# akashsengupta1997/indirect_learning_pose-shape

Hardware: AMD Instinct MI355X
Metric: meshes/sec fwd+bwd (SMPL->48x48 31-part seg) (higher is better)
Workload: dtype f32; 1 GPU; full decoder fwd+bwd (batch_smpl + projection + compute_mask + projects_to_seg), BASELINE configs[2]; meshes_per_gpu=128, global_batch=128, img_wh=48, vertex_sampling=1, verts=6890, params_per_mesh=86, launch=graph, steps_per_graph_launch=10, concurrent_chunks=1

## Files before the change

indirect_learning_pose-shape_amd/csrc/seg_bin.hip:

```cpp
#include "raster_common.h"

namespace smplr {
constexpr int BIN_Q0 = 3;
constexpr float X_ZERO = 104.0f;
constexpr float M_LOCAL = 208.0f;
#ifdef SMPLR_TL
constexpr int TL_BIN_WG = 128;
__device__ unsigned g_tl_bin[TL_BIN_WG * (BIN_T / 64) * 32];
#endif

struct Slot {
  int cls;
  int pos, pix;
  float u, v, m, x;
};

__device__ __forceinline__ Slot classify(float u, float v, float m, int pos, int W) {
  Slot s;
  s.pos = pos;
  s.u = u;
  s.v = v;
  s.m = m;
  s.cls = 1;
  s.pix = 0;
  s.x = 0.f;
  if (s.m > M_LOCAL) {
    s.cls = 0;
    const float c = rintf(s.u), r = rintf(s.v);
    if (c >= 0.0f && c <= (float)(W - 1) && r >= 0.0f && r <= (float)(W - 1)) {
      const float du = s.u - c, dv = s.v - r;
      s.x = __builtin_amdgcn_sqrtf(fmaf(du, du, dv * dv) * (s.m * s.m));
      if (s.x < X_ZERO) {
        s.cls = 2;
        s.pix = (int)r * W + (int)c;
      }
    }
  }
  return s;
}

template <bool VIS, bool STAGE, bool SKIN>
__global__ __launch_bounds__(BIN_T) void seg_bin_kernel(const float *__restrict__ proj,
                                                        float *__restrict__ mask,
                                                        const int *__restrict__ part_pos,
                                                        const int *__restrict__ part_off, int P, int K,
                                                        int VP, int W, int S, float4 *__restrict__ G,
                                                        int *__restrict__ goff, int *__restrict__ lstart,
                                                        uint2 *__restrict__ lrec, int vgrid, int ref_compat,
                                                        short *__restrict__ vslot, SkinIn sk) {
  extern __shared__ __attribute__((aligned(16))) int s_cnt[];
  __shared__ int s_poff[33], s_gstart[33], s_gpad[33], s_wave[BIN_T / 64], s_gb[BIN_T];
  __shared__ int s_any_empty, s_nonunit;
  __shared__ float4 sAj[SKIN ? 72 : 1];
  static_assert(!SKIN || (VIS && STAGE), "the skinning form is built for the decoder's path only");
  const int n = blockIdx.x, tid = threadIdx.x;
  SMPLR_TL_WAVE(g_tl_bin, BIN_T / 64, n, TL_BIN_WG)
  const int npix = W * W;
  const float *pj = proj + (size_t)n * VP * 3;
  float *mk = mask + (size_t)n * VP;
  const int cells = VIS ? vgrid * vgrid : 0, words = VIS ? (VP + 31) / 32 : 0;
  unsigned long long *zbuf = reinterpret_cast<unsigned long long *>(s_cnt + ((npix + 1) & ~1));
  unsigned int *vis = reinterpret_cast<unsigned int *>(zbuf + cells);
  float *sU = reinterpret_cast<float *>(vis + words), *sV = sU + VP;
  short *vsl = vslot ? vslot + (size_t)n * VP : nullptr;

  const int ipt = (K + BIN_T - 1) / BIN_T;
  const int k0 = tid * ipt, k1 = min(K, k0 + ipt);
  int pos[IPT_MAX];
  if (!SKIN) {
#pragma unroll
    for (int j = 0; j < IPT_MAX; ++j) pos[j] = (j < ipt) ? part_pos[min(k0 + j, K - 1)] : 0;
  }
  constexpr int VPT = SKIN ? 7 : 8;
  float vu[VPT], vv[VPT], vz[VPT];
  float4 tw[SKIN ? VPT : 1], tj[SKIN ? VPT : 1], aj = {0.f, 0.f, 0.f, 0.f};
  float c0 = 0.f, c1 = 0.f, c2 = 0.f, c3 = 0.f;
  if (SKIN) {
    aj = reinterpret_cast<const float4 *>(sk.A + (size_t)n * 288)[tid < 72 ? tid : 71];
    const float *c = sk.cam + (size_t)n * sk.x_stride;
    c0 = c[0]; c1 = c[1]; c2 = c[2]; c3 = c[3];
    const float *vp = sk.v_posed + (size_t)n * VP * 3;
#pragma unroll
    for (int q = 0; q < BIN_Q0; ++q) {
      const int v = min(tid + q * BIN_T, VP - 1);
      const float4 *tp = reinterpret_cast<const float4 *>(sk.top4 + (size_t)v * 8);
      tw[q] = tp[0];
      tj[q] = tp[1];
      vu[q] = vp[v * 3 + 0];
      vv[q] = vp[v * 3 + 1];
      vz[q] = vp[v * 3 + 2];
    }
  } else if (VIS || STAGE) {
#pragma unroll
    for (int q = 0; q < VPT; ++q) {
      const int v = min(tid + q * BIN_T, VP - 1);
      vu[q] = pj[v * 3 + 0];
      vv[q] = pj[v * 3 + 1];
      vz[q] = VIS ? pj[v * 3 + 2] : 0.0f;
    }
  }
  if (tid <= P) s_poff[tid] = part_off[tid];
  if (tid == 0) { s_nonunit = 0; s_any_empty = 0; }
  for (int i = tid; i < npix; i += BIN_T) s_cnt[i] = 0;
  if (vslot && !SKIN)
    for (int i = tid; i < VP; i += BIN_T) vsl[i] = -1;
  if (VIS) {
    for (int i = tid; i < cells; i += BIN_T) zbuf[i] = 0ull;
    for (int i = tid; i < words; i += BIN_T) vis[i] = 0u;
  }
  if (SKIN && tid < 72) sAj[tid] = aj;
  SMPLR_TL_STAMP(1);
  __syncthreads();
  SMPLR_TL_STAMP(2);
  if (SKIN) {
    const float *vp = sk.v_posed + (size_t)n * VP * 3;
#pragma unroll
    for (int q = BIN_Q0; q < VPT; ++q) {
      const int v = min(tid + q * BIN_T, VP - 1);
      const float4 *tp = reinterpret_cast<const float4 *>(sk.top4 + (size_t)v * 8);
      tw[q] = tp[0];
      tj[q] = tp[1];
      vu[q] = vp[v * 3 + 0];
      vv[q] = vp[v * 3 + 1];
      vz[q] = vp[v * 3 + 2];
    }
    if (vslot)
      for (int i = tid; i < VP; i += BIN_T) vsl[i] = -1;
    __builtin_amdgcn_sched_barrier(0);
    float *vo = sk.verts + (size_t)n * VP * 3, *po = sk.proj + (size_t)n * VP * 3;
#pragma unroll
    for (int q = 0; q < VPT; ++q) {
      const int v = tid + q * BIN_T;
      float T[12], X, Y, Z;
      skin_T_sparse(sAj, tw[q], tj[q], T);
      skin_apply(T, vu[q], vv[q], vz[q], X, Y, Z);
      vu[q] = project_u(X, c0, c2);
      vv[q] = project_u(Y, c1, c3);
      vz[q] = Z;
      if (v < VP) {
        if (sk.verts) { SMPLR_OUT_STORE(&vo[v * 3 + 0], X); SMPLR_OUT_STORE(&vo[v * 3 + 1], Y); SMPLR_OUT_STORE(&vo[v * 3 + 2], Z); }
        if (sk.proj) { SMPLR_OUT_STORE(&po[v * 3 + 0], vu[q]); SMPLR_OUT_STORE(&po[v * 3 + 1], vv[q]); SMPLR_OUT_STORE(&po[v * 3 + 2], Z); }
      }
      __builtin_amdgcn_sched_barrier(0);
    }
#pragma unroll
    for (int j = 0; j < IPT_MAX; ++j) pos[j] = (j < ipt) ? part_pos[min(k0 + j, K - 1)] : 0;
  }
  if (VIS || STAGE) {
    const float fG = (float)vgrid;
    for (int base = 0; base < VP; base += VPT * BIN_T) {
      if (base > 0) {
#pragma unroll
        for (int q = 0; q < VPT; ++q) {
          const int v = min(base + tid + q * BIN_T, VP - 1);
          vu[q] = pj[v * 3 + 0];
          vv[q] = pj[v * 3 + 1];
          vz[q] = VIS ? pj[v * 3 + 2] : 0.0f;
        }
      }
#pragma unroll
      for (int q = 0; q < VPT; ++q) {
        const int v = base + tid + q * BIN_T;
        if (v < VP) {
          if (STAGE) { sU[v] = vu[q]; sV[v] = vv[q]; }
          if (VIS) {
            const float pu = rintf(vu[q]);
            const float pv = rintf(vv[q]);
            if (pu >= 0.0f && pu < fG && pv >= 0.0f && pv < fG) {
              const int cell = (int)pv * vgrid + (int)pu;
              const unsigned long long key = ((unsigned long long)orderable(vz[q]) << 32) |
                                             (unsigned long long)(0xFFFFFFFFu - (unsigned)v);
              atomicMax(&zbuf[cell], key);
            }
          }
        }
      }
    }
    SMPLR_TL_STAMP(3);
    __syncthreads();
    SMPLR_TL_STAMP(4);
  }
  bool vertex1 = false;
  if (VIS) {
    int empty = 0;
    for (int i = tid; i < cells; i += BIN_T) {
      const unsigned long long key = zbuf[i];
      if (key == 0ull) {
        empty = 1;
      } else {
        const unsigned int v = 0xFFFFFFFFu - (unsigned int)(key & 0xFFFFFFFFull);
        atomicOr(&vis[v >> 5], 1u << (v & 31));
      }
    }
    if (empty) s_any_empty = 1;
    SMPLR_TL_STAMP(5);
    __syncthreads();
    SMPLR_TL_STAMP(6);
    vertex1 = s_any_empty && ref_compat && VP > 1;
    if (mask)
      for (int v = tid; v < VP; v += BIN_T)
        SMPLR_OUT_STORE(&mk[v], (((vis[v >> 5] >> (v & 31)) & 1u) || (vertex1 && v == 1)) ? 1.0f : 500.0f);
  }
  SMPLR_TL_STAMP(7);
  float4 *Gn = G + (size_t)n * S;
  int *goffn = goff + (size_t)n * goff_stride(P);
  int *lstartn = lstart + (size_t)n * (npix + 1);
  uint2 *lrecn = lrec + (size_t)n * K;

  Slot sl[IPT_MAX];
  int gcnt = 0;
  unsigned gbits = 0;
#pragma unroll
  for (int j = 0; j < IPT_MAX; ++j) {
    const int k = k0 + j;
    sl[j].cls = 0;
    if (j < ipt && k < k1) {
      const int ps = pos[j];
      const float m = VIS ? ((((vis[ps >> 5] >> (ps & 31)) & 1u) || (vertex1 && ps == 1)) ? 1.0f : 500.0f) : mk[ps];
      const float u = STAGE ? sU[ps] : pj[ps * 3], v = STAGE ? sV[ps] : pj[ps * 3 + 1];
      sl[j] = classify(u, v, m, ps, W);
    }
    if (sl[j].cls == 1) {
      ++gcnt;
      gbits |= 1u << j;
      if (sl[j].m != 1.0f) s_nonunit = 1;
    } else if (sl[j].cls == 2) {
      atomicAdd(&s_cnt[sl[j].pix], 1);
    }
  }
  int p0 = 0;
  if (k0 < k1) {
    int lo = 0, hi = P;
    while (hi - lo > 1) {
      const int mid = (lo + hi) >> 1;
      if (s_poff[mid] <= k0) lo = mid; else hi = mid;
    }
    p0 = lo;
  }
  SMPLR_TL_STAMP(8);
  __syncthreads();
  SMPLR_TL_STAMP(9);
  const int ept = (npix + BIN_T - 1) / BIN_T;
  const int e0 = tid * ept, e1 = min(npix, e0 + ept);
  int loc = 0;
  for (int e = e0; e < e1; ++e) loc += s_cnt[e];
  int tot2;
  const int base2 = block_excl_scan(gcnt | (loc << 16), s_wave, &tot2);
  const int gbase = base2 & 0xffff, gtotal = tot2 & 0xffff, ltotal = tot2 >> 16;
  SMPLR_TL_STAMP(10);
  s_gb[tid] = gbase | (int)(gbits << 16);
  {
    int run = base2 >> 16;
    for (int e = e0; e < e1; ++e) {
      const int c = s_cnt[e];
      s_cnt[e] = run;
      lstartn[e] = run;
      run += c;
    }
    if (tid == 0) lstartn[npix] = ltotal;
  }
  SMPLR_TL_STAMP(11);
  __syncthreads();
  SMPLR_TL_STAMP(12);
  if (tid < 128) {
    const int l = tid & 63;
    int gs = gtotal;
    const int kk = s_poff[l <= P ? l : P];
    if (l < P && kk < K) {
      const int t = kk / ipt, j = kk - t * ipt;
      const int w = s_gb[t];
      gs = (w & 0xffff) + __popc(((unsigned)w >> 16) & ((1u << j) - 1u));
    }
    const int gnext = __shfl_down(gs, 1, 64);
    const int cnt = (l < P) ? (gnext - gs + GP - 1) / GP * GP : 0;
    if (tid < 64) {
      int inc = cnt;
#pragma unroll
      for (int o = 1; o < 32; o <<= 1) {
        const int t = __shfl_up(inc, o, 64);
        if (tid >= o) inc += t;
      }
      if (tid <= P) {
        s_gstart[tid] = gs;
        s_gpad[tid] = inc - cnt;
        goffn[tid] = inc - cnt;
      }
    } else {
      const int key = l < P ? ((cnt << 5) | (31 - l)) : -1;
      int rank = 0;
#pragma unroll
      for (int q = 0; q < 31; ++q) rank += (__builtin_amdgcn_readlane(key, q) > key) ? 1 : 0;
      if (l < P) goffn[P + 2 + rank] = l;
    }
  }
  SMPLR_TL_STAMP(13);
  __syncthreads();
  SMPLR_TL_STAMP(14);
  {
    int p = p0;
    int run = gbase;
#pragma unroll
    for (int j = 0; j < IPT_MAX; ++j) {
      const int k = k0 + j;
      if (!(j < ipt && k < k1)) continue;
      while (k >= s_poff[p + 1]) ++p;
      const Slot s = sl[j];
      if (s.cls == 1) {
        const int slot = s_gpad[p] + (run - s_gstart[p]);
        Gn[slot] = make_float4(s.u, s.v, s.m * s.m, __int_as_float(s.pos));
        if (vslot) vsl[s.pos] = (short)slot;
        ++run;
      } else if (s.cls == 2) {
        const int dst = atomicAdd(&s_cnt[s.pix], 1);
        lrecn[dst] = make_uint2(__float_as_uint(s.x), (unsigned)p);
        Gn[s_gpad[P] + dst] = make_float4(s.u, s.v, s.m * s.m, __int_as_float(s.pos));
        if (vslot) vsl[s.pos] = (short)(s_gpad[P] + dst);
      }
    }
  }
  SMPLR_TL_STAMP(15);
  if (tid == 0) goffn[P + 1] = s_nonunit;
  if (tid == 0)
    Gn[S - 1] = make_float4(__int_as_float(s_gpad[P] + lstartn[npix]), __int_as_float(s_nonunit), __int_as_float(s_gpad[P]),
                            __int_as_float(-1));
  if (tid < P) {
    const int cnt = s_gstart[tid + 1] - s_gstart[tid];
    for (int i = s_gpad[tid] + cnt; i < s_gpad[tid + 1]; ++i)
      Gn[i] = make_float4(INFINITY, INFINITY, 1.0f, __int_as_float(-1));
  }
  SMPLR_TL_STAMP(16);
  SMPLR_TL_STAMP(17);
  SMPLR_TL_STAMP(18);
}

struct BinLds { size_t base, total; bool stage; };
static BinLds bin_lds(int VP, int W, int grid_wh ) {
  BinLds b;
  b.base = (size_t)((W * W + 1) & ~1) * sizeof(int);
  if (grid_wh > 0) b.base += (size_t)grid_wh * grid_wh * 8 + (size_t)((VP + 31) / 32) * 4;
  b.stage = b.base + (size_t)VP * 8 <= 150 * 1024;
  b.total = b.base + (b.stage ? (size_t)VP * 8 : 0);
  return b;
}

int seg_bin_impl(const char *fn, const float *proj, float *mask, bool fuse_vis, int grid_wh, int ref_compat, int B, int VP,
                 int W, const int32_t *part_pos, const int32_t *part_off, int P, int K, void *workspace, float *rec,
                 int16_t *vslot, void *stream, SkinIn sk) {
  SMPLR_REQUIRE(B >= 0 && VP > 0 && VP <= 32767 && W > 0 && W <= 160 && P >= 1 && P <= 31 && K > 0 && K <= BIN_T * IPT_MAX,
                "%s: bad sizes B=%d VP=%d W=%d (max 160) P=%d (max 31) K=%d", fn, B, VP, W, P, K);
  SMPLR_REQUIRE(!fuse_vis || (grid_wh > 0 && grid_wh <= 128), "%s: bad grid_wh=%d (max 128)", fn, grid_wh);
  if (B == 0) return 0;
  const bool skin = sk.v_posed != nullptr;
  SMPLR_REQUIRE((skin || (proj && mask)) && part_pos && part_off && workspace && rec, "%s: null pointer", fn);
  SMPLR_REQUIRE(!skin || (sk.top4 && sk.A && sk.cam && sk.x_stride >= 4 && sk.proj == proj && fuse_vis &&
                          VP <= 7 * BIN_T),
                "%s: the skinning form needs the sparse weights, A, camera rows, the fused mask and V <= %d",
                fn, 7 * BIN_T);
  hipStream_t st = as_stream(stream);
  const SegWs ws = seg_ws_layout(B, W, P, K);
  const int S = seg_slots(P, K);
  char *base = reinterpret_cast<char *>(workspace);
  float4 *G = reinterpret_cast<float4 *>(rec);
  int *goff = reinterpret_cast<int *>(base + ws.goff_off);
  int *lstart = reinterpret_cast<int *>(base + ws.lstart_off);
  uint2 *lrec = reinterpret_cast<uint2 *>(base + ws.lrec_off);
  const BinLds bl = bin_lds(VP, W, fuse_vis ? grid_wh : 0);
  SMPLR_REQUIRE(bl.base <= 150 * 1024, "%s: pixel counters + grid + flags need %zu B of LDS (max 153600)", fn, bl.base);
  const bool stage = bl.stage;
  const size_t lds = bl.total;
#define SMPLR_BIN_LAUNCH(VIS_, STAGE_, SKIN_)                                                                 \
  {                                                                                                           \
    int rc = lds_attr<&seg_bin_kernel<VIS_, STAGE_, SKIN_>>(lds);          \
    if (rc) return rc;                                                                                        \
    hipLaunchKernelGGL((seg_bin_kernel<VIS_, STAGE_, SKIN_>), dim3(B), dim3(BIN_T), lds, st, proj, mask,      \
                       part_pos, part_off, P, K, VP, W, S, G, goff, lstart, lrec, fuse_vis ? grid_wh : 1,     \
                       ref_compat, reinterpret_cast<short *>(vslot), sk);                                     \
  }
  SMPLR_REQUIRE(!skin || stage, "%s: the skinning form needs the staged (u, v) to fit LDS", fn);
  if (skin) SMPLR_BIN_LAUNCH(true, true, true)
  else if (fuse_vis && stage) SMPLR_BIN_LAUNCH(true, true, false)
  else if (fuse_vis) SMPLR_BIN_LAUNCH(true, false, false)
  else if (stage) SMPLR_BIN_LAUNCH(false, true, false)
  else SMPLR_BIN_LAUNCH(false, false, false)
#undef SMPLR_BIN_LAUNCH
  SMPLR_LAUNCH_CHECK(fn);
  return 0;
}
}

extern "C" {

int smplr_seg_slots(int P, int K) { return (P > 0 && K > 0) ? smplr::seg_slots(P, K) : 0; }

size_t smplr_seg_workspace(int B, int VP, int W, int P, int K) {
  if (B <= 0 || VP <= 0 || W <= 0 || P <= 0 || K <= 0) return 0;
  return smplr::seg_ws_layout(B, W, P, K).total;
}

int smplr_seg_bin(const float *proj, float *mask, int B, int VP, int W, int grid_wh, int ref_compat,
                  const int32_t *part_pos, const int32_t *part_off, int P, int K, void *workspace, float *rec,
                  int16_t *vslot, void *stream) {
  return smplr::seg_bin_impl("smplr_seg_bin", proj, mask, grid_wh > 0, grid_wh, ref_compat, B, VP, W, part_pos,
                             part_off, P, K, workspace, rec, vslot, stream);
}

int smplr_skin_vis_seg_fits(int V, int W, int grid_wh) {
  if (V <= 0 || V > 7 * smplr::BIN_T || W <= 0 || W > 160 || grid_wh <= 0 || grid_wh > 128) return 0;
  const smplr::BinLds b = smplr::bin_lds(V, W, grid_wh);
  return (b.base <= 150 * 1024 && b.stage) ? 1 : 0;
}

}

#ifdef SMPLR_TL
SMPLR_TL_EXPORT(bin, smplr::g_tl_bin, smplr::TL_BIN_WG * (smplr::BIN_T / 64) * 32)
#endif
```

indirect_learning_pose-shape_amd/csrc/skin.hip:

```cpp
#include "common.h"

namespace smplr {

typedef float f32x4 __attribute__((ext_vector_type(4)));

constexpr int SK_MB = 1;
constexpr int SKB_T = 256;

template <bool SPARSE>
__global__ __launch_bounds__(256) void skin_fwd_kernel(const float *__restrict__ v_posed,
                                                       const float *__restrict__ lbs,
                                                       const float *__restrict__ top4,
                                                       const float *__restrict__ A,
                                                       const float *__restrict__ cam, int x_stride,
                                                       int B, int V, int vs, int VP,
                                                       float *__restrict__ verts,
                                                       float *__restrict__ proj) {
  __shared__ float4 sAj[SPARSE ? 72 : 1];
  const int v = blockIdx.x * 256 + threadIdx.x;
  const bool live = v < V;
  const int vc = live ? v : V - 1;
  float w[SPARSE ? 1 : 24];
  float4 ww = {0.f, 0.f, 0.f, 0.f}, jj = {0.f, 0.f, 0.f, 0.f};
  if (SPARSE) {
// ... 141 lines not shown
    if (slot >= 0) { gp0 += sx; gp1 += sy; }
  }
  if (tid < 72) sAj[tid] = aj;
  SMPLR_TL_STAMP(1);
  __syncthreads();
  SMPLR_TL_STAMP(2);

  const int cr = li >> 2, cc = li & 3;

  {
    const bool proj_on = live && has_proj && sampled;
    float g0 = 0.f, g1 = 0.f, g2 = 0.f;
    float dku = 0.f, dkv = 0.f, du0 = 0.f, dv0 = 0.f;
    if (live) { g0 = gv0; g1 = gv1; g2 = gv2; }
    if (proj_on) { g0 = fmaf(ck0, gp0, g0); g1 = fmaf(ck1, gp1, g1); g2 += gp2; du0 = gp0; dv0 = gp1; }
    float dp0 = 0.f, dp1 = 0.f, dp2 = 0.f;
#pragma unroll
    for (int r = 0; r < 3; ++r) {
      float t0 = 0.f, t1 = 0.f, t2 = 0.f, t3 = 0.f;
#pragma unroll
      for (int jq = 0; jq < (SPARSE ? 4 : 24); ++jq) {
        const int j = SPARSE ? jx[jq & 3] : jq;
        const float wj = SPARSE ? w4[jq & 3] : w[SPARSE ? 0 : jq];
        const float4 rr = sAj[j * 3 + r];
        t0 = fmaf(wj, rr.x, t0); t1 = fmaf(wj, rr.y, t1); t2 = fmaf(wj, rr.z, t2); t3 = fmaf(wj, rr.w, t3);
      }
      const float gr = r == 0 ? g0 : (r == 1 ? g1 : g2);
      dp0 = fmaf(t0, gr, dp0); dp1 = fmaf(t1, gr, dp1); dp2 = fmaf(t2, gr, dp2);
      if (r < 2 && proj_on) {
        const float XY = fmaf(t2, p2, fmaf(t1, p1, fmaf(t0, p0, t3)));
        if (r == 0) dku = XY * gp0; else dkv = XY * gp1;
      }
    }
    if (live) {
      float *o = dv_posed + ((size_t)n * V + v) * 3;
      o[0] = dp0; o[1] = dp1; o[2] = dp2;
    }
    SMPLR_TL_STAMP(3);
    float wa0[8], wa1[8];
    const __amdgpu_buffer_rsrc_t rs =
        __builtin_amdgcn_make_buffer_rsrc(const_cast<float *>(lbs), 0, V * 24 * 4, 0x00020000);
    const int vb = blockIdx.x * SKB_T + wave * 64 + lk;
    const int o0 = (vb * 24 + li) * 4, o1 = (vb * 24 + 16 + (li & 7)) * 4;
    {
  #pragma unroll
      for (int sI = 0; sI < 8; ++sI) {
        wa0[sI] = __builtin_bit_cast(float, __builtin_amdgcn_raw_buffer_load_b32(rs, o0 + sI * 384, 0, 0));
        wa1[sI] = __builtin_bit_cast(float, __builtin_amdgcn_raw_buffer_load_b32(rs, o1 + sI * 384, 0, 0));
      }
    }
    sG[tid][0] = g0; sG[tid][1] = g1; sG[tid][2] = g2; sG[tid][3] = 0.f;
    sP[tid][0] = p0; sP[tid][1] = p1; sP[tid][2] = p2; sP[tid][3] = 1.0f;
    __syncthreads();
    SMPLR_TL_STAMP(4);

    f32x4 acc0 = {0.f, 0.f, 0.f, 0.f}, acc1 = {0.f, 0.f, 0.f, 0.f};
#pragma unroll
    for (int s = 0; s < 16; ++s) {
      const int t = wave * 64 + s * 4 + lk;
      const float a0 = wa0[s & 7];
      const float a1 = (li < 8) ? wa1[s & 7] : 0.0f;
      const float b = (li < 12) ? sG[t][cr] * sP[t][cc] : 0.0f;
      acc0 = __builtin_amdgcn_mfma_f32_16x16x4f32(a0, b, acc0, 0, 0, 0);
      acc1 = __builtin_amdgcn_mfma_f32_16x16x4f32(a1, b, acc1, 0, 0, 0);
      if (s < 8) {
        wa0[s] = __builtin_bit_cast(float, __builtin_amdgcn_raw_buffer_load_b32(rs, o0 + (s + 8) * 384, 0, 0));
        wa1[s] = __builtin_bit_cast(float, __builtin_amdgcn_raw_buffer_load_b32(rs, o1 + (s + 8) * 384, 0, 0));
      }
    }
    SMPLR_TL_STAMP(5);
    if (li < 12) {
#pragma unroll
      for (int r = 0; r < 4; ++r) {
        const int j0 = lk * 4 + r;
        sRed[wave][j0 * 12 + li] = acc0[r];
        if (j0 < 8) sRed[wave][(16 + j0) * 12 + li] = acc1[r];
      }
    }
    const float r0 = wave_sum(dku), r1 = wave_sum(dkv), r2 = wave_sum(du0), r3 = wave_sum(dv0);
    if (lane == 0) {
      sRed[wave][288] = r0; sRed[wave][289] = r1; sRed[wave][290] = r2; sRed[wave][291] = r3;
    }
    __syncthreads();
    SMPLR_TL_STAMP(6);
    for (int e = tid; e < SKB_PART; e += SKB_T) {
      float acc = 0.f;
#pragma unroll
      for (int wv = 0; wv < SKB_T / 64; ++wv) acc += sRed[wv][e];
      part[((size_t)n * gridDim.x + blockIdx.x) * SKB_PART + e] = acc;
    }
    SMPLR_TL_STAMP(7);
  }
}

__global__ __launch_bounds__(320) void skin_bwd_reduce_kernel(const float *__restrict__ part, int nblk,
                                                              float *__restrict__ dA,
                                                              float *__restrict__ dcam) {
  const int n = blockIdx.x, e = threadIdx.x;
  if (e >= SKB_PART) return;
  float acc = 0.f;
  for (int b = 0; b < nblk; ++b) acc += part[((size_t)n * nblk + b) * SKB_PART + e];
  if (e < 288) dA[(size_t)n * 288 + e] = acc;
  else if (dcam) dcam[(size_t)n * 4 + (e - 288)] = acc;
}

__global__ __launch_bounds__(256) void project_fwd_kernel(const float *__restrict__ verts,
                                                          const float *__restrict__ cam, int x_stride,
                                                          int V, int vs, int VP, float *__restrict__ proj) {
  const int n = blockIdx.y, i = blockIdx.x * 256 + threadIdx.x;
  if (i >= VP) return;
  const float *c = cam + (size_t)n * x_stride;
  const float *p = verts + ((size_t)n * V + (size_t)i * vs) * 3;
  float *o = proj + ((size_t)n * VP + i) * 3;
  o[0] = c[2] + p[0] * c[0];
  o[1] = c[3] + p[1] * c[1];
  o[2] = p[2];
}

__global__ __launch_bounds__(256) void project_bwd_kernel(const float *__restrict__ dproj,
                                                          const float *__restrict__ verts,
                                                          const float *__restrict__ cam, int x_stride,
                                                          int V, int vs, int VP, float *__restrict__ dverts,
                                                          float *__restrict__ dcam) {
  __shared__ float red[4][4];
  const int n = blockIdx.x, tid = threadIdx.x;
  const float *c = cam + (size_t)n * x_stride;
  const float ku = c[0], kv = c[1];
  float s0 = 0.f, s1 = 0.f, s2 = 0.f, s3 = 0.f;
  for (int v = tid; v < V; v += 256) {
    float *o = dverts + ((size_t)n * V + v) * 3;
    if (vs <= 1 || v % vs == 0) {
      const float *d = dproj + ((size_t)n * VP + (vs <= 1 ? v : v / vs)) * 3;
      const float *p = verts + ((size_t)n * V + v) * 3;
      const float du = d[0], dv = d[1];
      o[0] = ku * du; o[1] = kv * dv; o[2] = d[2];
      s0 += p[0] * du; s1 += p[1] * dv; s2 += du; s3 += dv;
    } else {
      o[0] = 0.f; o[1] = 0.f; o[2] = 0.f;
    }
  }
  s0 = wave_sum(s0); s1 = wave_sum(s1); s2 = wave_sum(s2); s3 = wave_sum(s3);
  if ((tid & 63) == 0) {
    red[tid >> 6][0] = s0; red[tid >> 6][1] = s1; red[tid >> 6][2] = s2; red[tid >> 6][3] = s3;
  }
  __syncthreads();
  if (tid < 4) dcam[(size_t)n * 4 + tid] = red[0][tid] + red[1][tid] + red[2][tid] + red[3][tid];
}

#ifdef SMPLR_TL
constexpr int TL_SKINREC_WG = 896;
__device__ unsigned g_tl_skinrec[TL_SKINREC_WG * 4 * 32];
#endif
constexpr int SKR_T = 256;
constexpr int SKR_VPT = 4;
constexpr int SKR_CHUNK = SKR_T * SKR_VPT;

__global__ __launch_bounds__(SKR_T) __attribute__((amdgpu_waves_per_eu(4, 8))) void skin_bwd_rec_kernel(
    const float *__restrict__ v_posed, const float *__restrict__ top4,
    const float *__restrict__ A, const float *__restrict__ cam, int x_stride, int B, int V, int vs, int VP,
    float *__restrict__ dv_posed, float *__restrict__ part, const float *__restrict__ seg_part,
    const short *__restrict__ seg_vslot, int seg_nsplit) {
  __shared__ float sG[SKR_T][4];
  __shared__ float sP[SKR_T][4];
  __shared__ float4 sW[SKR_T];
  __shared__ float4 sJ[SKR_T];
  __shared__ float sRed[SKR_T / 64][SKB_PART];
  __shared__ float4 sAj[72];
  __shared__ int sVid[SKR_CHUNK];
  __shared__ short sSlot[SKR_CHUNK];
  __shared__ int sCnt[SKR_VPT * (SKR_T / 64)];
  const int tid = threadIdx.x, wave = tid >> 6, lane = tid & 63;
  const int n = blockIdx.y, v0 = blockIdx.x * SKR_CHUNK;
  SMPLR_TL_WAVE(g_tl_skinrec, SKR_T / 64, blockIdx.y * gridDim.x + blockIdx.x, TL_SKINREC_WG)
  const float4 aj = reinterpret_cast<const float4 *>(A + (size_t)n * 288)[tid < 72 ? tid : 71];
  const float *cm = cam + (size_t)n * x_stride;
  const float ck0 = cm[0], ck1 = cm[1];
  int slot[SKR_VPT];
#pragma unroll
  for (int i = 0; i < SKR_VPT; ++i) {
    const int v = v0 + i * SKR_T + tid;
    const bool sampled = v < V && ((vs <= 1) || (v % vs == 0));
    const int vpi = (vs <= 1) ? v : v / vs;
    slot[i] = seg_vslot[(size_t)n * VP + min(vpi, VP - 1)];
    if (!sampled) slot[i] = -1;
  }
  if (tid < 72) sAj[tid] = aj;
  SMPLR_TL_STAMP(1);
  int pre[SKR_VPT];
#pragma unroll
  for (int i = 0; i < SKR_VPT; ++i) {
    const unsigned long long m = __ballot(slot[i] >= 0);
    pre[i] = __popcll(m & ((1ull << lane) - 1ull));
    if (lane == 0) sCnt[i * (SKR_T / 64) + wave] = __popcll(m);
  }
  SMPLR_TL_STAMP(2);
  __syncthreads();
  SMPLR_TL_STAMP(3);
  int R = 0;
  {
    int base[SKR_VPT] = {0, 0, 0, 0};
#pragma unroll
    for (int k = 0; k < SKR_VPT * (SKR_T / 64); ++k) {
      const int c = sCnt[k];
#pragma unroll
      for (int i = 0; i < SKR_VPT; ++i)
        if (k < i * (SKR_T / 64) + wave) base[i] += c;
      R += c;
    }
#pragma unroll
    for (int i = 0; i < SKR_VPT; ++i) {
      const int v = v0 + i * SKR_T + tid;
      if (slot[i] >= 0) {
        sVid[base[i] + pre[i]] = v;
        sSlot[base[i] + pre[i]] = (short)slot[i];
      }
    }
  }
  SMPLR_TL_STAMP(4);
  __syncthreads();
  SMPLR_TL_STAMP(5);
  const int li = lane & 15, lk = lane >> 4;
  const int cr = li >> 2, cc = li & 3;
  const float fl0 = (float)li, fl1 = (float)(16 + li);
  f32x4 acc0 = {0.f, 0.f, 0.f, 0.f}, acc1 = {0.f, 0.f, 0.f, 0.f};
  float dku = 0.f, dkv = 0.f, du0 = 0.f, dv0 = 0.f;
  for (int r0 = 0; r0 < R; r0 += SKR_T) {
    const int idx = r0 + tid;
    const bool valid = idx < R;
    const int vid = sVid[min(idx, R - 1)], sl = sSlot[min(idx, R - 1)];
    const float4 *tp = reinterpret_cast<const float4 *>(top4 + (size_t)vid * 8);
    const float4 ww = tp[0], jj = tp[1];
    const float *vp = v_posed + ((size_t)n * V + vid) * 3;
    const float p0 = vp[0], p1 = vp[1], p2 = vp[2];
    const int win = sl / SB_SLOTS;
    const float *sp = seg_part + ((size_t)n * seg_nsplit * SB_NWIN + win) * (SB_SLOTS * 2) + (sl - win * SB_SLOTS) * 2;
    float sx = 0.0f, sy = 0.0f;
    if (seg_nsplit <= 2) {
      const float2 t0 = *reinterpret_cast<const float2 *>(sp);
      const float2 t1 = *reinterpret_cast<const float2 *>(sp + (size_t)(seg_nsplit - 1) * (SB_NWIN * SB_SLOTS * 2));
      sx = t0.x + (seg_nsplit > 1 ? t1.x : 0.0f);
      sy = t0.y + (seg_nsplit > 1 ? t1.y : 0.0f);
    } else {
      constexpr int GC = 6;
      for (int s0 = 0; s0 < seg_nsplit; s0 += GC) {
        float2 t[GC];
#pragma unroll
        for (int u = 0; u < GC; ++u)
          t[u] = *reinterpret_cast<const float2 *>(sp + (size_t)min(s0 + u, seg_nsplit - 1) * (SB_NWIN * SB_SLOTS * 2));
#pragma unroll
        for (int u = 0; u < GC; ++u) {
          sx += (s0 + u < seg_nsplit) ? t[u].x : 0.0f;
          sy += (s0 + u < seg_nsplit) ? t[u].y : 0.0f;
        }
      }
    }
    const float gp0 = valid ? sx : 0.0f, gp1 = valid ? sy : 0.0f;
    const float g0 = fmaf(ck0, gp0, 0.0f), g1 = fmaf(ck1, gp1, 0.0f);
    const float w4[4] = {ww.x, ww.y, ww.z, ww.w};
    const int jx[4] = {(int)jj.x, (int)jj.y, (int)jj.z, (int)jj.w};
    float dp0 = 0.f, dp1 = 0.f, dp2 = 0.f;
#pragma unroll
    for (int r = 0; r < 2; ++r) {
      float t0 = 0.f, t1 = 0.f, t2 = 0.f, t3 = 0.f;
#pragma unroll
      for (int jq = 0; jq < 4; ++jq) {
        const float4 rr = sAj[jx[jq] * 3 + r];
        t0 = fmaf(w4[jq], rr.x, t0); t1 = fmaf(w4[jq], rr.y, t1); t2 = fmaf(w4[jq], rr.z, t2); t3 = fmaf(w4[jq], rr.w, t3);
      }
      const float gr = r == 0 ? g0 : g1;
      dp0 = fmaf(t0, gr, dp0); dp1 = fmaf(t1, gr, dp1); dp2 = fmaf(t2, gr, dp2);
      const float XY = fmaf(t2, p2, fmaf(t1, p1, fmaf(t0, p0, t3)));
      if (r == 0) dku += XY * gp0; else dkv += XY * gp1;
    }
    du0 += gp0;
    dv0 += gp1;
    sG[tid][0] = g0; sG[tid][1] = g1; sG[tid][2] = 0.f; sG[tid][3] = 0.f;
    sP[tid][0] = p0; sP[tid][1] = p1; sP[tid][2] = p2; sP[tid][3] = 1.0f;
    sW[tid] = valid ? ww : make_float4(0.f, 0.f, 0.f, 0.f);
    sJ[tid] = jj;
    SMPLR_TL_STAMP(6);
    __syncthreads();
    SMPLR_TL_STAMP(7);
    if (r0 + wave * 64 < R) {
#pragma unroll
      for (int s = 0; s < 16; ++s) {
        const int t = wave * 64 + s * 4 + lk;
        const float4 wq = sW[t], jq = sJ[t];
        const float a0 = ((jq.x == fl0 ? wq.x : 0.0f) + (jq.y == fl0 ? wq.y : 0.0f)) +
                         ((jq.z == fl0 ? wq.z : 0.0f) + (jq.w == fl0 ? wq.w : 0.0f));
        const float a1 = ((jq.x == fl1 ? wq.x : 0.0f) + (jq.y == fl1 ? wq.y : 0.0f)) +
                         ((jq.z == fl1 ? wq.z : 0.0f) + (jq.w == fl1 ? wq.w : 0.0f));
        const float b = (li < 12) ? sG[t][cr] * sP[t][cc] : 0.0f;
        acc0 = __builtin_amdgcn_mfma_f32_16x16x4f32(a0, b, acc0, 0, 0, 0);
        acc1 = __builtin_amdgcn_mfma_f32_16x16x4f32(li < 8 ? a1 : 0.0f, b, acc1, 0, 0, 0);
      }
    }
    if (valid) {
      float *o = dv_posed + ((size_t)n * V + vid) * 3;
      o[0] = dp0; o[1] = dp1; o[2] = dp2;
    }
    SMPLR_TL_STAMP(8);
    __syncthreads();
  }
#pragma unroll
  for (int i = 0; i < SKR_VPT; ++i) {
    const int v = v0 + i * SKR_T + tid;
    if (slot[i] < 0 && v < V) {
      float *o = dv_posed + ((size_t)n * V + v) * 3;
      o[0] = 0.0f; o[1] = 0.0f; o[2] = 0.0f;
    }
  }
  SMPLR_TL_STAMP(9);
  if (li < 12) {
#pragma unroll
    for (int r = 0; r < 4; ++r) {
      const int j0 = lk * 4 + r;
      sRed[wave][j0 * 12 + li] = acc0[r];
      if (j0 < 8) sRed[wave][(16 + j0) * 12 + li] = acc1[r];
    }
  }
  const float q0 = wave_sum(dku), q1 = wave_sum(dkv), q2 = wave_sum(du0), q3 = wave_sum(dv0);
  if (lane == 0) {
    sRed[wave][288] = q0; sRed[wave][289] = q1; sRed[wave][290] = q2; sRed[wave][291] = q3;
  }
  __syncthreads();
  SMPLR_TL_STAMP(10);
  for (int e = tid; e < SKB_PART; e += SKR_T) {
    float acc = 0.f;
#pragma unroll
    for (int wv = 0; wv < SKR_T / 64; ++wv) acc += sRed[wv][e];
    part[((size_t)n * gridDim.x + blockIdx.x) * SKB_PART + e] = acc;
  }
  SMPLR_TL_STAMP(11);
#ifdef SMPLR_TL
  if (tl__) tl__[12] = (unsigned)R;
#endif
}

int skin_bwd_nblk(int V) { return (V + SKB_T - 1) / SKB_T; }

int launch_skin_bwd_partials(const float *dverts, const float *dproj, SegGrad sg, const float *v_posed,
                             const float *lbs_weights, const float *lbs_top4, const float *A, const float *cam,
                             int x_stride, int B, int V, int vs, float *dv_posed, float *part, hipStream_t st,
                             int *nblk_out) {
  const int VP = (V + vs - 1) / vs;
  static const bool rec_on = !(getenv("SMPLR_SKIN_BWD_REC") && atoi(getenv("SMPLR_SKIN_BWD_REC")) == 0);
  if (rec_on && !dverts && !dproj && sg.part && lbs_top4) {
    const dim3 grid((V + SKR_CHUNK - 1) / SKR_CHUNK, B);
    hipLaunchKernelGGL(skin_bwd_rec_kernel, grid, dim3(SKR_T), 0, st, v_posed, lbs_top4, A, cam, x_stride, B, V, vs, VP,
                       dv_posed, part, sg.part, reinterpret_cast<const short *>(sg.vslot), sg.nsplit);
    SMPLR_LAUNCH_CHECK("skin_bwd_rec_kernel");
    *nblk_out = (int)grid.x;
    return 0;
  }
  *nblk_out = skin_bwd_nblk(V);
  const dim3 grid(skin_bwd_nblk(V), (B + SKB_MB - 1) / SKB_MB);
  if (lbs_top4)
    hipLaunchKernelGGL(skin_bwd_kernel<true>, grid, dim3(SKB_T), 0, st, dverts, dproj, v_posed, lbs_weights, lbs_top4,
                       A, cam, x_stride, B, V, vs, VP, dv_posed, part, sg.part, reinterpret_cast<const short *>(sg.vslot),
                       sg.nsplit);
  else
    hipLaunchKernelGGL(skin_bwd_kernel<false>, grid, dim3(SKB_T), 0, st, dverts, dproj, v_posed, lbs_weights, lbs_top4,
                       A, cam, x_stride, B, V, vs, VP, dv_posed, part, sg.part, reinterpret_cast<const short *>(sg.vslot),
                       sg.nsplit);
  SMPLR_LAUNCH_CHECK("skin_bwd_kernel");
  return 0;
}

}

extern "C" {

static int check_vs(int V, int vs) { return vs >= 1 && vs <= V; }

int smplr_skin_fwd(const float *v_posed, const float *lbs_weights, const float *lbs_top4, const float *A,
                   const float *cam, int x_stride, int B, int V, int vertex_sampling, float *verts,
                   float *proj, void *stream) {
  using namespace smplr;
  SMPLR_REQUIRE(B >= 0 && V > 0 && check_vs(V, vertex_sampling), "smplr_skin_fwd: bad sizes B=%d V=%d vs=%d",
                B, V, vertex_sampling);
  if (B == 0) return 0;
  SMPLR_REQUIRE(v_posed && lbs_weights && A && (verts || proj), "smplr_skin_fwd: null pointer");
  SMPLR_REQUIRE(!proj || (cam && x_stride >= 4), "smplr_skin_fwd: proj requested without camera rows");
  const int VP = (V + vertex_sampling - 1) / vertex_sampling;
  dim3 grid((V + 255) / 256, (B + SK_MB - 1) / SK_MB);
  if (lbs_top4)
    hipLaunchKernelGGL(skin_fwd_kernel<true>, grid, dim3(256), 0, as_stream(stream), v_posed, lbs_weights, lbs_top4, A,
                       cam, x_stride, B, V, vertex_sampling, VP, verts, proj);
  else
    hipLaunchKernelGGL(skin_fwd_kernel<false>, grid, dim3(256), 0, as_stream(stream), v_posed, lbs_weights, lbs_top4, A,
                       cam, x_stride, B, V, vertex_sampling, VP, verts, proj);
  SMPLR_LAUNCH_CHECK("smplr_skin_fwd");
  return 0;
}

size_t smplr_skin_bwd_workspace(int B, int V) {
  using namespace smplr;
  if (B <= 0 || V <= 0) return 0;
  return (size_t)B * ((V + SKB_T - 1) / SKB_T) * SKB_PART * sizeof(float);
}

int smplr_skin_bwd(const float *dverts, const float *dproj, const float *v_posed,
                   const float *lbs_weights, const float *lbs_top4, const float *A, const float *cam,
                   int x_stride, int B, int V,
                   int vertex_sampling, float *dv_posed, float *dA, float *dcam, void *workspace,
                   void *stream) {
  using namespace smplr;
  SMPLR_REQUIRE(B >= 0 && V > 0 && check_vs(V, vertex_sampling), "smplr_skin_bwd: bad sizes B=%d V=%d vs=%d",
                B, V, vertex_sampling);
  if (B == 0) return 0;
  SMPLR_REQUIRE(v_posed && lbs_weights && A && dv_posed && dA && workspace, "smplr_skin_bwd: null pointer");
  SMPLR_REQUIRE(dverts || dproj, "smplr_skin_bwd: need dverts and/or dproj");
  SMPLR_REQUIRE(!dproj || (cam && x_stride >= 4), "smplr_skin_bwd: dproj given without camera rows");
  int nblk = 0;
  int rc = launch_skin_bwd_partials(dverts, dproj, SegGrad{nullptr, nullptr, 0}, v_posed, lbs_weights, lbs_top4, A, cam,
                                    x_stride, B, V, vertex_sampling, dv_posed, reinterpret_cast<float *>(workspace),
                                    as_stream(stream), &nblk);
  if (rc) return rc;
  hipLaunchKernelGGL(skin_bwd_reduce_kernel, dim3(B), dim3(320), 0, as_stream(stream),
                     reinterpret_cast<const float *>(workspace), nblk, dA, dcam);
  SMPLR_LAUNCH_CHECK("smplr_skin_bwd(reduce)");
  return 0;
}

int smplr_project_fwd(const float *verts, const float *cam, int x_stride, int B, int V,
                      int vertex_sampling, float *proj, void *stream) {
  using namespace smplr;
  SMPLR_REQUIRE(B >= 0 && V > 0 && check_vs(V, vertex_sampling) && x_stride >= 4,
                "smplr_project_fwd: bad sizes B=%d V=%d vs=%d x_stride=%d", B, V, vertex_sampling, x_stride);
  if (B == 0) return 0;
  SMPLR_REQUIRE(verts && cam && proj, "smplr_project_fwd: null pointer");
  const int VP = (V + vertex_sampling - 1) / vertex_sampling;
  hipLaunchKernelGGL(project_fwd_kernel, dim3((VP + 255) / 256, B), dim3(256), 0, as_stream(stream), verts,
                     cam, x_stride, V, vertex_sampling, VP, proj);
  SMPLR_LAUNCH_CHECK("smplr_project_fwd");
  return 0;
}

int smplr_project_bwd(const float *dproj, const float *verts, const float *cam, int x_stride, int B, int V,
                      int vertex_sampling, float *dverts, float *dcam, void *stream) {
  using namespace smplr;
  SMPLR_REQUIRE(B >= 0 && V > 0 && check_vs(V, vertex_sampling) && x_stride >= 4,
                "smplr_project_bwd: bad sizes B=%d V=%d vs=%d x_stride=%d", B, V, vertex_sampling, x_stride);
  if (B == 0) return 0;
  SMPLR_REQUIRE(dproj && verts && cam && dverts && dcam, "smplr_project_bwd: null pointer");
  const int VP = (V + vertex_sampling - 1) / vertex_sampling;
  hipLaunchKernelGGL(project_bwd_kernel, dim3(B), dim3(256), 0, as_stream(stream), dproj, verts, cam,
                     x_stride, V, vertex_sampling, VP, dverts, dcam);
  SMPLR_LAUNCH_CHECK("smplr_project_bwd");
  return 0;
}

}

#ifdef SMPLR_TL
SMPLR_TL_EXPORT(skin, smplr::g_tl_skin, smplr::TL_SKIN_WG * (smplr::SKB_T / 64) * 32)
SMPLR_TL_EXPORT(skinrec, smplr::g_tl_skinrec, smplr::TL_SKINREC_WG * 4 * 32)
#endif
```

Baseline: 1.063 million meshes/s.

## Split skinned vertex/projection output stores into separate workgroups in seg_bin

When the batch fits in half the CUs, the skinning bin kernel launches 2*B workgroups. The second half only recomputes skinning and projection and writes the verts/proj outputs, while the first half does the binning without those global stores. This takes the output-store traffic off the critical binning workgroups and runs it on otherwise idle CUs. The cost is duplicated skinning work. LDS is padded to at least 80KB, presumably to keep the two roles on separate CUs. An env var can override the choice.

```diff
diff --git a/indirect_learning_pose-shape_amd/csrc/seg_bin.hip b/indirect_learning_pose-shape_amd/csrc/seg_bin.hip
--- a/indirect_learning_pose-shape_amd/csrc/seg_bin.hip
+++ b/indirect_learning_pose-shape_amd/csrc/seg_bin.hip
@@ -5,7 +5,7 @@
 constexpr float X_ZERO = 104.0f;
 constexpr float M_LOCAL = 208.0f;
 #ifdef SMPLR_TL
-constexpr int TL_BIN_WG = 128;
+constexpr int TL_BIN_WG = 256;
 __device__ unsigned g_tl_bin[TL_BIN_WG * (BIN_T / 64) * 32];
 #endif
 
@@ -39,7 +39,44 @@
   return s;
 }
 
-template <bool VIS, bool STAGE, bool SKIN>
+__device__ __forceinline__ void seg_bin_outputs(const SkinIn &sk, int n, int VP, float4 *sAj) {
+  constexpr int VPT = 7;
+  const int tid = threadIdx.x;
+  const float4 aj = reinterpret_cast<const float4 *>(sk.A + (size_t)n * 288)[tid < 72 ? tid : 71];
+  const float *c = sk.cam + (size_t)n * sk.x_stride;
+  const float c0 = c[0], c1 = c[1], c2 = c[2], c3 = c[3];
+  const float *vp = sk.v_posed + (size_t)n * VP * 3;
+  float4 tw[VPT], tj[VPT];
+  float p0[VPT], p1[VPT], p2[VPT];
+#pragma unroll
+  for (int q = 0; q < VPT; ++q) {
+    const int v = min(tid + q * BIN_T, VP - 1);
+    const float4 *tp = reinterpret_cast<const float4 *>(sk.top4 + (size_t)v * 8);
+    tw[q] = tp[0];
+    tj[q] = tp[1];
+    p0[q] = vp[v * 3 + 0];
+    p1[q] = vp[v * 3 + 1];
+    p2[q] = vp[v * 3 + 2];
+  }
+  if (tid < 72) sAj[tid] = aj;
+  __syncthreads();
+  float *vo = sk.verts + (size_t)n * VP * 3, *po = sk.proj + (size_t)n * VP * 3;
+#pragma unroll
+  for (int q = 0; q < VPT; ++q) {
+    const int v = tid + q * BIN_T;
+    float T[12], X, Y, Z;
+    skin_T_sparse(sAj, tw[q], tj[q], T);
+    skin_apply(T, p0[q], p1[q], p2[q], X, Y, Z);
+    const float pu = project_u(X, c0, c2), pv = project_u(Y, c1, c3);
+    if (v < VP) {
+      if (sk.verts) { SMPLR_OUT_STORE(&vo[v * 3 + 0], X); SMPLR_OUT_STORE(&vo[v * 3 + 1], Y); SMPLR_OUT_STORE(&vo[v * 3 + 2], Z); }
+      if (sk.proj) { SMPLR_OUT_STORE(&po[v * 3 + 0], pu); SMPLR_OUT_STORE(&po[v * 3 + 1], pv); SMPLR_OUT_STORE(&po[v * 3 + 2], Z); }
+    }
+    __builtin_amdgcn_sched_barrier(0);
+  }
+}
+
+template <bool VIS, bool STAGE, bool SKIN, bool ROLES = false>
 __global__ __launch_bounds__(BIN_T) void seg_bin_kernel(const float *__restrict__ proj,
                                                         float *__restrict__ mask,
                                                         const int *__restrict__ part_pos,
@@ -53,8 +90,14 @@
   __shared__ int s_any_empty, s_nonunit;
   __shared__ float4 sAj[SKIN ? 72 : 1];
   static_assert(!SKIN || (VIS && STAGE), "the skinning form is built for the decoder's path only");
+  static_assert(!ROLES || SKIN, "the output role belongs to the skinning form");
   const int n = blockIdx.x, tid = threadIdx.x;
   SMPLR_TL_WAVE(g_tl_bin, BIN_T / 64, n, TL_BIN_WG)
+  if (ROLES && n >= (int)(gridDim.x >> 1)) {
+    seg_bin_outputs(sk, n - (int)(gridDim.x >> 1), VP, sAj);
+    SMPLR_TL_STAMP(18);
+    return;
+  }
   const int npix = W * W;
   const float *pj = proj + (size_t)n * VP * 3;
   float *mk = mask + (size_t)n * VP;
@@ -137,10 +180,11 @@
       vu[q] = project_u(X, c0, c2);
       vv[q] = project_u(Y, c1, c3);
       vz[q] = Z;
-      if (v < VP) {
+      if (!ROLES && v < VP) {
         if (sk.verts) { SMPLR_OUT_STORE(&vo[v * 3 + 0], X); SMPLR_OUT_STORE(&vo[v * 3 + 1], Y); SMPLR_OUT_STORE(&vo[v * 3 + 2], Z); }
         if (sk.proj) { SMPLR_OUT_STORE(&po[v * 3 + 0], vu[q]); SMPLR_OUT_STORE(&po[v * 3 + 1], vv[q]); SMPLR_OUT_STORE(&po[v * 3 + 2], Z); }
       }
+      if (ROLES) asm volatile("" : "+v"(vu[q]), "+v"(vv[q]), "+v"(vz[q]));
       __builtin_amdgcn_sched_barrier(0);
     }
 #pragma unroll
@@ -341,6 +385,20 @@
   b.stage = b.base + (size_t)VP * 8 <= 150 * 1024;
   b.total = b.base + (b.stage ? (size_t)VP * 8 : 0);
   return b;
+}
+
+constexpr size_t ROLES_LDS = 80 * 1024 + 16;
+static bool bin_roles(int B) {
+  if (const char *e = getenv("SMPLR_BIN_ROLES"))
+    if (*e) return atoi(e) != 0;
+  static int cus[64] = {};
+  int dev = 0, n = 0;
+  if (hipGetDevice(&dev) != hipSuccess) return false;
+  const bool known = dev >= 0 && dev < 64;
+  if (known && cus[dev] > 0) return 2 * (long long)B <= cus[dev];
+  if (hipDeviceGetAttribute(&n, hipDeviceAttributeMultiprocessorCount, dev) != hipSuccess || n <= 0) return false;
+  if (known) cus[dev] = n;
+  return 2 * (long long)B <= n;
 }
 
 int seg_bin_impl(const char *fn, const float *proj, float *mask, bool fuse_vis, int grid_wh, int ref_compat, int B, int VP,
@@ -368,20 +426,22 @@
   SMPLR_REQUIRE(bl.base <= 150 * 1024, "%s: pixel counters + grid + flags need %zu B of LDS (max 153600)", fn, bl.base);
   const bool stage = bl.stage;
   const size_t lds = bl.total;
-#define SMPLR_BIN_LAUNCH(VIS_, STAGE_, SKIN_)                                                                 \
+#define SMPLR_BIN_LAUNCH(GRID_, LDS_, ...)                                                                    \
   {                                                                                                           \
-    int rc = lds_attr<&seg_bin_kernel<VIS_, STAGE_, SKIN_>>(lds);          \
+    int rc = lds_attr<&seg_bin_kernel<__VA_ARGS__>>(LDS_);                                                    \
     if (rc) return rc;                                                                                        \
-    hipLaunchKernelGGL((seg_bin_kernel<VIS_, STAGE_, SKIN_>), dim3(B), dim3(BIN_T), lds, st, proj, mask,      \
+    hipLaunchKernelGGL((seg_bin_kernel<__VA_ARGS__>), dim3(GRID_), dim3(BIN_T), LDS_, st, proj, mask,         \
                        part_pos, part_off, P, K, VP, W, S, G, goff, lstart, lrec, fuse_vis ? grid_wh : 1,     \
                        ref_compat, reinterpret_cast<short *>(vslot), sk);                                     \
   }
   SMPLR_REQUIRE(!skin || stage, "%s: the skinning form needs the staged (u, v) to fit LDS", fn);
-  if (skin) SMPLR_BIN_LAUNCH(true, true, true)
-  else if (fuse_vis && stage) SMPLR_BIN_LAUNCH(true, true, false)
-  else if (fuse_vis) SMPLR_BIN_LAUNCH(true, false, false)
-  else if (stage) SMPLR_BIN_LAUNCH(false, true, false)
-  else SMPLR_BIN_LAUNCH(false, false, false)
+  const size_t lds2 = lds > ROLES_LDS ? lds : ROLES_LDS;
+  if (skin && (sk.verts || sk.proj) && bin_roles(B)) SMPLR_BIN_LAUNCH(2 * B, lds2, true, true, true, true)
+  else if (skin) SMPLR_BIN_LAUNCH(B, lds, true, true, true)
+  else if (fuse_vis && stage) SMPLR_BIN_LAUNCH(B, lds, true, true, false)
+  else if (fuse_vis) SMPLR_BIN_LAUNCH(B, lds, true, false, false)
+  else if (stage) SMPLR_BIN_LAUNCH(B, lds, false, true, false)
+  else SMPLR_BIN_LAUNCH(B, lds, false, false, false)
 #undef SMPLR_BIN_LAUNCH
   SMPLR_LAUNCH_CHECK(fn);
   return 0;
```

Measured after the change: 1.035 million meshes/s. 0.973x the previous value.

## Prefetch seg-gradient sums before compaction and skip zero-gradient vertices in skin backward

Applied to the files above, without the earlier changes.

The per-vertex seg_part gradient gather now happens before the stream-compaction step rather than inside the main loop. By default, vertices whose summed gradient is exactly zero are dropped from the compacted work list and simply get zeroed dv_posed, which shrinks the MFMA accumulation loop. Shared memory is cut by aliasing sRed onto the sW/sJ buffers, storing vertex ids as 16-bit offsets and storing the sums in place of slots, and the waves_per_eu minimum rises from 4 to 5. Because every vertex's gather is now issued up front, loads are spent on vertices that turn out to be skipped, and the higher occupancy target may cause register spills.

```diff
diff --git a/indirect_learning_pose-shape_amd/csrc/skin.hip b/indirect_learning_pose-shape_amd/csrc/skin.hip
--- a/indirect_learning_pose-shape_amd/csrc/skin.hip
+++ b/indirect_learning_pose-shape_amd/csrc/skin.hip
@@ -317,22 +317,27 @@
 __device__ unsigned g_tl_skinrec[TL_SKINREC_WG * 4 * 32];
 #endif
 constexpr int SKR_T = 256;
-constexpr int SKR_VPT = 4;
+#ifndef SMPLR_SKR_VPT
+#define SMPLR_SKR_VPT 4
+#endif
+constexpr int SKR_VPT = SMPLR_SKR_VPT;
 constexpr int SKR_CHUNK = SKR_T * SKR_VPT;
 
-__global__ __launch_bounds__(SKR_T) __attribute__((amdgpu_waves_per_eu(4, 8))) void skin_bwd_rec_kernel(
+__global__ __launch_bounds__(SKR_T) __attribute__((amdgpu_waves_per_eu(5, 8))) void skin_bwd_rec_kernel(
     const float *__restrict__ v_posed, const float *__restrict__ top4,
     const float *__restrict__ A, const float *__restrict__ cam, int x_stride, int B, int V, int vs, int VP,
     float *__restrict__ dv_posed, float *__restrict__ part, const float *__restrict__ seg_part,
-    const short *__restrict__ seg_vslot, int seg_nsplit) {
+    const short *__restrict__ seg_vslot, int seg_nsplit, int live_only) {
   __shared__ float sG[SKR_T][4];
   __shared__ float sP[SKR_T][4];
-  __shared__ float4 sW[SKR_T];
-  __shared__ float4 sJ[SKR_T];
-  __shared__ float sRed[SKR_T / 64][SKB_PART];
+  __shared__ float4 sWJ[2 * SKR_T];
+  float4 *sW = sWJ;
+  float4 *sJ = sWJ + SKR_T;
+  float (*sRed)[SKB_PART] = reinterpret_cast<float (*)[SKB_PART]>(sWJ);
+  static_assert(sizeof(float) * (SKR_T / 64) * SKB_PART <= sizeof(float4) * 2 * SKR_T, "sRed inside sWJ");
   __shared__ float4 sAj[72];
-  __shared__ int sVid[SKR_CHUNK];
-  __shared__ short sSlot[SKR_CHUNK];
+  __shared__ unsigned short sVid[SKR_CHUNK];
+  __shared__ float2 sSum[SKR_CHUNK];
   __shared__ int sCnt[SKR_VPT * (SKR_T / 64)];
   const int tid = threadIdx.x, wave = tid >> 6, lane = tid & 63;
   const int n = blockIdx.y, v0 = blockIdx.x * SKR_CHUNK;
@@ -351,19 +356,52 @@
   }
   if (tid < 72) sAj[tid] = aj;
   SMPLR_TL_STAMP(1);
+  float sx[SKR_VPT], sy[SKR_VPT];
+#pragma unroll
+  for (int i = 0; i < SKR_VPT; ++i) {
+    const int sl = max(slot[i], 0);
+    const int win = sl / SB_SLOTS;
+    const float *sp = seg_part + ((size_t)n * seg_nsplit * SB_NWIN + win) * (SB_SLOTS * 2) + (sl - win * SB_SLOTS) * 2;
+    sx[i] = 0.0f; sy[i] = 0.0f;
+    if (seg_nsplit <= 2) {
+      const float2 t0 = *reinterpret_cast<const float2 *>(sp);
+      const float2 t1 = *reinterpret_cast<const float2 *>(sp + (size_t)(seg_nsplit - 1) * (SB_NWIN * SB_SLOTS * 2));
+      sx[i] = t0.x + (seg_nsplit > 1 ? t1.x : 0.0f);
+      sy[i] = t0.y + (seg_nsplit > 1 ? t1.y : 0.0f);
+    } else {
+      constexpr int GC = 6;
+      for (int s0 = 0; s0 < seg_nsplit; s0 += GC) {
+        float2 t[GC];
+#pragma unroll
+        for (int u = 0; u < GC; ++u)
+          t[u] = *reinterpret_cast<const float2 *>(sp + (size_t)min(s0 + u, seg_nsplit - 1) * (SB_NWIN * SB_SLOTS * 2));
+#pragma unroll
+        for (int u = 0; u < GC; ++u) {
+          sx[i] += (s0 + u < seg_nsplit) ? t[u].x : 0.0f;
+          sy[i] += (s0 + u < seg_nsplit) ? t[u].y : 0.0f;
+        }
+      }
+    }
+  }
+  unsigned livem = 0, zerom = 0;
   int pre[SKR_VPT];
 #pragma unroll
   for (int i = 0; i < SKR_VPT; ++i) {
-    const unsigned long long m = __ballot(slot[i] >= 0);
+    const bool live = slot[i] >= 0 && !(live_only && sx[i] == 0.0f && sy[i] == 0.0f);
+    const unsigned long long m = __ballot(live);
     pre[i] = __popcll(m & ((1ull << lane) - 1ull));
     if (lane == 0) sCnt[i * (SKR_T / 64) + wave] = __popcll(m);
+    if (live) livem |= 1u << i;
+    else if (v0 + i * SKR_T + tid < V) zerom |= 1u << i;
   }
   SMPLR_TL_STAMP(2);
   __syncthreads();
   SMPLR_TL_STAMP(3);
   int R = 0;
   {
-    int base[SKR_VPT] = {0, 0, 0, 0};
+    int base[SKR_VPT];
+#pragma unroll
+    for (int i = 0; i < SKR_VPT; ++i) base[i] = 0;
 #pragma unroll
     for (int k = 0; k < SKR_VPT * (SKR_T / 64); ++k) {
       const int c = sCnt[k];
@@ -374,10 +412,9 @@
     }
 #pragma unroll
     for (int i = 0; i < SKR_VPT; ++i) {
-      const int v = v0 + i * SKR_T + tid;
-      if (slot[i] >= 0) {
-        sVid[base[i] + pre[i]] = v;
-        sSlot[base[i] + pre[i]] = (short)slot[i];
+      if (livem >> i & 1u) {
+        sVid[base[i] + pre[i]] = (unsigned short)(i * SKR_T + tid);
+        sSum[base[i] + pre[i]] = make_float2(sx[i], sy[i]);
       }
     }
   }
@@ -392,34 +429,13 @@
   for (int r0 = 0; r0 < R; r0 += SKR_T) {
     const int idx = r0 + tid;
     const bool valid = idx < R;
-    const int vid = sVid[min(idx, R - 1)], sl = sSlot[min(idx, R - 1)];
+    const int vid = v0 + sVid[min(idx, R - 1)];
+    const float2 sm = sSum[min(idx, R - 1)];
     const float4 *tp = reinterpret_cast<const float4 *>(top4 + (size_t)vid * 8);
     const float4 ww = tp[0], jj = tp[1];
     const float *vp = v_posed + ((size_t)n * V + vid) * 3;
     const float p0 = vp[0], p1 = vp[1], p2 = vp[2];
-    const int win = sl / SB_SLOTS;
-    const float *sp = seg_part + ((size_t)n * seg_nsplit * SB_NWIN + win) * (SB_SLOTS * 2) + (sl - win * SB_SLOTS) * 2;
-    float sx = 0.0f, sy = 0.0f;
-    if (seg_nsplit <= 2) {
-      const float2 t0 = *reinterpret_cast<const float2 *>(sp);
-      const float2 t1 = *reinterpret_cast<const float2 *>(sp + (size_t)(seg_nsplit - 1) * (SB_NWIN * SB_SLOTS * 2));
-      sx = t0.x + (seg_nsplit > 1 ? t1.x : 0.0f);
-      sy = t0.y + (seg_nsplit > 1 ? t1.y : 0.0f);
-    } else {
-      constexpr int GC = 6;
-      for (int s0 = 0; s0 < seg_nsplit; s0 += GC) {
-        float2 t[GC];
-#pragma unroll
-        for (int u = 0; u < GC; ++u)
-          t[u] = *reinterpret_cast<const float2 *>(sp + (size_t)min(s0 + u, seg_nsplit - 1) * (SB_NWIN * SB_SLOTS * 2));
-#pragma unroll
-        for (int u = 0; u < GC; ++u) {
-          sx += (s0 + u < seg_nsplit) ? t[u].x : 0.0f;
-          sy += (s0 + u < seg_nsplit) ? t[u].y : 0.0f;
-        }
-      }
-    }
-    const float gp0 = valid ? sx : 0.0f, gp1 = valid ? sy : 0.0f;
+    const float gp0 = valid ? sm.x : 0.0f, gp1 = valid ? sm.y : 0.0f;
     const float g0 = fmaf(ck0, gp0, 0.0f), g1 = fmaf(ck1, gp1, 0.0f);
     const float w4[4] = {ww.x, ww.y, ww.z, ww.w};
     const int jx[4] = {(int)jj.x, (int)jj.y, (int)jj.z, (int)jj.w};
@@ -470,7 +486,7 @@
 #pragma unroll
   for (int i = 0; i < SKR_VPT; ++i) {
     const int v = v0 + i * SKR_T + tid;
-    if (slot[i] < 0 && v < V) {
+    if (zerom >> i & 1u) {
       float *o = dv_posed + ((size_t)n * V + v) * 3;
       o[0] = 0.0f; o[1] = 0.0f; o[2] = 0.0f;
     }
@@ -510,10 +526,11 @@
                              int *nblk_out) {
   const int VP = (V + vs - 1) / vs;
   static const bool rec_on = !(getenv("SMPLR_SKIN_BWD_REC") && atoi(getenv("SMPLR_SKIN_BWD_REC")) == 0);
+  static const bool live_on = !(getenv("SMPLR_SKIN_BWD_LIVE") && atoi(getenv("SMPLR_SKIN_BWD_LIVE")) == 0);
   if (rec_on && !dverts && !dproj && sg.part && lbs_top4) {
     const dim3 grid((V + SKR_CHUNK - 1) / SKR_CHUNK, B);
     hipLaunchKernelGGL(skin_bwd_rec_kernel, grid, dim3(SKR_T), 0, st, v_posed, lbs_top4, A, cam, x_stride, B, V, vs, VP,
-                       dv_posed, part, sg.part, reinterpret_cast<const short *>(sg.vslot), sg.nsplit);
+                       dv_posed, part, sg.part, reinterpret_cast<const short *>(sg.vslot), sg.nsplit, live_on ? 1 : 0);
     SMPLR_LAUNCH_CHECK("skin_bwd_rec_kernel");
     *nblk_out = (int)grid.x;
     return 0;
```

New measurement: 1.059 million meshes/s before, 1.089 million meshes/s after, median of 6. 2.8% higher.
